# DaehwanKimLab/hisat2

Hardware: AMD Instinct MI355X
Metric: reads/sec, 101 bp PE, REDUCED-SIZE (256000000 bp, GRCh38 contig profile) linear index, --no-spliced-alignment: HI_Aligner::go per pair on the GPU (inputs and report events resident in HBM), SAM-identical to hisat2 (higher is better)
Workload: dtype u32

## Files before the change

### hisat2_amd/csrc/h2g_fast.h

```cpp
#pragma once
#include "h2g_align.h"
#ifndef FG_GRAPH
#define FG_GRAPH 0
#endif
#if FG_GRAPH
#include "h2g_graph.h"
#endif
#ifndef FG_SPLICED
#define FG_SPLICED 0
#endif
#if FG_SPLICED && (FG_GRAPH || FG_ALIGN_MATE)
#error "FG_SPLICED is built for linear indexes, without alignMate in the pass"
#endif

namespace h2g {

#define FG_FE     4
#define FG_HW     (6 + FG_FE / 2 + FG_GRAPH * FG_FE)
#define FG_LW     3
#define FG_NLONG  3
#define FG_NLONGC 3
#define FG_NLONGT (FG_NLONG + FG_NLONGC)
#define FG_NCO    5
#define FG_NRES   2
// ... 129 lines not shown
#define F_SMIN16 (-32768)
#define F_SMAX16 32767
H2G_HD uint32_t fs_rl(const FState& S, uint32_t m) { return m ? S.rl1 : S.rl0; }
H2G_HD uint32_t fs_ro(const FState& S, uint32_t m) { return m ? S.ro1 : S.ro0; }
H2G_HD uint32_t fs_nres(const FState& S, uint32_t m) { return m ? S.nres1 : S.nres0; }
H2G_HD uint32_t fs_nsearched(const FState& S, uint32_t m) { return m ? S.nsearched1 : S.nsearched0; }
H2G_HD int32_t fs_bestUnp(const FState& S, uint32_t m) { return m ? S.bestUnp1 : S.bestUnp0; }
H2G_HD int32_t fs_minsc(const FState& S, uint32_t m) { return m ? S.minsc1 : S.minsc0; }
H2G_HD uint32_t fs_b4(uint32_t w, uint32_t x) { return (w >> (8 * x)) & 0xffu; }
H2G_HD uint32_t fs_b4_set(uint32_t w, uint32_t x, uint32_t v) { return (w & ~(0xffu << (8 * x))) | ((v & 0xffu) << (8 * x)); }
H2G_HD uint32_t fs_sumsq(const FState& S, uint32_t x) { return x == 0 ? S.rb_sumsq0 : x == 1 ? S.rb_sumsq1 : x == 2 ? S.rb_sumsq2 : S.rb_sumsq3; }
H2G_HD void fs_sumsq_add(FState& S, uint32_t x, uint32_t v) { if(x == 0) S.rb_sumsq0 += v; else if(x == 1) S.rb_sumsq1 += v; else if(x == 2) S.rb_sumsq2 += v; else S.rb_sumsq3 += v; }
#define F_SMIN INT32_MIN

struct FCtx {
	const DGfm* g; const DRef* ref; const DLocalSet* ls; const AlnParams* P;
	DReads rd[2];
	const uint32_t* pk[2]; uint32_t pk_stride;
	const char* name[2]; uint32_t namelen[2];
	int64_t* sc; uint32_t sc_stride;
	FastOut O;
	uint32_t defer_slow = 0;
	uint32_t mate_handover = 0;
#if FG_GRAPH
	const DAlts* alts;
	GraphWS* gws;
#endif
#if FG_SPLICED
	const DSpliceDB* ssdb = nullptr;
	uint32_t rdid_base = 0;
#endif
};
#if FG_GRAPH
#define FG_IE_NOFIT 0xffffffffu
H2G_HD uint32_t fg_ie_pack(const IEdges& ie) {
	if(ie.n > 2) return FG_IE_NOFIT;
	uint32_t w = ie.n;
	if(ie.n > 0) { if(ie.e[0][0] > 127 || ie.e[0][1] > 127) return FG_IE_NOFIT; w |= (ie.e[0][0] << 2) | (ie.e[0][1] << 9); }
	if(ie.n > 1) { if(ie.e[1][0] > 127 || ie.e[1][1] > 127) return FG_IE_NOFIT; w |= (ie.e[1][0] << 16) | (ie.e[1][1] << 23); }
	return w;
}
H2G_HD void fg_ie_unpack(uint32_t w, IEdges* ie) {
	ie->n = w & 3u;
	ie->e[0][0] = (w >> 2) & 127u; ie->e[0][1] = (w >> 9) & 127u;
	ie->e[1][0] = (w >> 16) & 127u; ie->e[1][1] = (w >> 23) & 127u;
}
// ... 512 lines not shown
	const uint32_t ro = rd.offs[i], rl = rd.offs[i + 1] - ro;
	if(rl > H2G_PK_MAXLEN) return false;
	const uint8_t* src = rd.codes + ro;
	uint32_t anyn = 0;
	for(uint32_t w = 0; w < H2G_PK_WORDS; w++) {
		uint32_t bits = 0;
		if(w * 16 < rl) {
			for(uint32_t q = 0; q < 4; q++) {
				const uint32_t at = w * 16 + q * 4;
				if(at >= rl) break;
				uint32_t four;
				memcpy(&four, src + at, 4);
				const uint32_t left = rl - at;
				if(left < 4) four &= (1u << (8 * left)) - 1u;
				anyn |= four & 0x04040404u;
				const uint32_t lo = four & 0x03030303u;
				bits |= ((lo | (lo >> 6) | (lo >> 12) | (lo >> 18)) & 0xffu) << (8 * q);
			}
		}
		pk[w * stride] = bits;
	}
	return anyn == 0;
}
H2G_HD uint32_t fg_res_base(uint32_t m, uint32_t k) { return FW_RES + (m * FG_NRES + k) * 3; }
H2G_HD uint32_t fg_res_hit(uint32_t m, uint32_t k) { return FW_RH + (m * FG_NRES + k) * FG_HW; }

H2G_HD uint32_t fg_rand_seed(const FCtx& C, const FState& S, uint32_t set) {
	uint32_t rseed = C.P->seed0;
	const uint32_t len = fs_rl(S, set);
	const uint32_t* pk = set ? C.pk[1] : C.pk[0];
	for(uint32_t w = 0; w < H2G_PK_WORDS; w++) rseed ^= pk[w * C.pk_stride];
	const char* quals = set ? C.rd[1].quals : C.rd[0].quals;
	if(quals) {
		const char* q = quals + fs_ro(S, set);
		for(uint32_t i = 0; i < len; i++) rseed ^= ((uint32_t)q[i] << ((i & 3) << 3));
	} else {
		for(uint32_t b = 0; b < 4; b++) if(((len + 3 - b) >> 2) & 1u) rseed ^= (uint32_t)'I' << (b << 3);
	}
	const char* name = set ? C.name[1] : C.name[0];
	const uint32_t namelen = set ? C.namelen[1] : C.namelen[0];
	for(uint32_t i = 0; i < namelen; i++) {
		const int p = name[i];
		if(p == '/') break;
		rseed ^= ((uint32_t)p << ((i & 3) << 3));
	}
	return rseed;
// ... 155 lines not shown
		if(rdi < 0) F_GOTO(FPC_AFTER_LOOP);
		const uint32_t x = (uint32_t)rdi * 2 + (uint32_t)fwi, xr = (uint32_t)rdi * 2 + (uint32_t)(1 - fwi);
		{
			const uint32_t numSearched = fs_b4(S.rb_nps, x) - fs_b4(S.rb_nus, x);
			const int32_t bestScore = fs_bestUnp(S, rdi), msc = fs_minsc(S, rdi);
			if(bestScore >= msc) {
				const uint32_t maxmm = (uint32_t)((-(int64_t)bestScore + sc.mmpMax - 1) / sc.mmpMax);
				if(numSearched > maxmm + 1) {
					S.rb_done |= 1u << x; fg_pool_free(W, S, x);
					if(S.paired) {
						const int32_t ob = fs_bestUnp(S, 1 - rdi), om = fs_minsc(S, 1 - rdi);
						if(ob >= om && S.npairs > 0) F_GOTO(FPC_AFTER_LOOP); else F_GOTO(FPC_NB_PICK);
					} else F_GOTO(FPC_AFTER_LOOP);
				}
			}
			if(((S.rb_done >> xr) & 1u) && bestScore < msc) {
				const uint32_t rcs = fs_b4(S.rb_nps, xr) - fs_b4(S.rb_nus, xr);
				if(numSearched > rcs + (P.anchorStop ? 1u : 0u)) { S.rb_done |= 1u << x; fg_pool_free(W, S, x); F_GOTO(FPC_AFTER_LOOP); }
			}
		}
		S.nb_rdi = rdi; S.nb_fwi = fwi;
		S.sv_rdi = (uint32_t)rdi; S.sv_fw = fwi == 0;
		S.a0 = fs_b4(S.rb_cur, x);
		F_OP(FOP_PSEARCH, FPC_NB_AFTER_PS);
	}
	case FPC_NB_AFTER_PS: {
		const int rdi = S.nb_rdi, fwi = S.nb_fwi;
		const uint32_t x = (uint32_t)rdi * 2 + (uint32_t)fwi;
		const uint32_t top = S.a0, bot = S.a1, len = S.a2 & 0xffu, type = (S.a2 >> 8) & 0xffu, done = (S.a2 >> 16) & 1u, anchor = (S.a2 >> 17) & 1u, nus = S.a2 >> 18;
		{ const uint32_t nr_ = S.nrank + (S.a4 & 0xffffu), ns_ = S.nside + (S.a4 >> 16); if(nr_ > 0xffffu || ns_ > 0xffffu) F_BAIL(FB_OTHER); S.nrank = nr_; S.nside = ns_; }
		S.rb_nps = fs_b4_set(S.rb_nps, x, fs_b4(S.rb_nps, x) + 1); S.rb_nus = fs_b4_set(S.rb_nus, x, fs_b4(S.rb_nus, x) + nus); S.rb_cur = fs_b4_set(S.rb_cur, x, S.a3);
		const uint32_t np = fs_b4(S.rb_np, x);
		if(np >= 16) F_BAIL(FB_PARTIAL);
		fs_sumsq_add(S, x, len * len);
		if(bot > top && bot != H2G_MAX) {
			S.rb_nonempty |= 1u << x;
			if(len > minK + 2) {
				uint32_t k = 0;
				for(; k < FG_NLONG; k++) if(W.ld(FW_LONG + FG_LW * k + 2) == 0) break;
				if(k >= FG_NLONG) {
					for(; k < FG_NLONGT; k++) if(!((S.pool_x >> (k - FG_NLONG)) & 1u)) break;
					if(k >= FG_NLONGT) F_BAIL(FB_LONGPOOL);
					S.pool_x = S.pool_x | (1u << (k - FG_NLONG));
				}
				W.st(fg_pool(k), top); W.st(fg_pool(k) + 1, bot);
#if FG_GRAPH
// ... 1031 lines not shown
	case FPC_DONE:
	case FPC_BAIL:
	default: return;
	}
}
#undef F_GOTO
#undef F_OP
#undef F_RC_RET
#undef F_RC_CALL
#undef F_MINSC_LIVE

H2G_HD void fast_op_psearch(const FCtx& C, FState& S) {
	const AlnParams& P = *C.P;
	h2g_fm_hit fh;
#if FG_GRAPH
	IEdges ie;
	partial_search_graph_item(*C.g, fg_sv(C, S), S.a0, P.pseudogeneStop != 0, P.anchorStop != 0, P.khits, P.kseeds, &fh, &ie);
	S.a6 = fh.node_top; S.a7 = fh.node_bot; S.a8 = fg_ie_pack(ie);
#else
	partial_search_item(*C.g, fg_sv(C, S), S.a0, P.pseudogeneStop != 0, P.anchorStop != 0, P.khits, &fh);
#endif
	S.a5 = S.a0;
	S.a0 = fh.top; S.a1 = fh.bot;
	S.a2 = (fh.len & 0xffu) | (fh.hit_type << 8) | ((fh.done ? 1u : 0u) << 16) | ((fh.anchorStop ? 1u : 0u) << 17) | (fh.numUniqueSearch << 18);
	S.a3 = fh.cur; S.a4 = (fh.nrank & 0xffffu) | (fh.nside << 16);
}
#ifndef FG_WALK_STEPS
#define FG_WALK_STEPS 20
#endif
#ifndef FG_LWALK_STEPS
#define FG_LWALK_STEPS 10
#endif
#if FG_GRAPH
H2G_HD bool fast_op_gcoords(const FCtx& C, FState& S, const FWords& W) {
	if(!(S.a4 & 2u)) {
		uint32_t nelt = S.a7 - S.a6;
		if(nelt > S.a2) nelt = S.a2;
		if(nelt == 1 && S.a1 - S.a0 == 1) { S.a4 |= 2u; S.a2 = 0; }
	}
	if(S.a4 & 2u) {
		uint32_t row = S.a0, node = S.a6, steps = S.a2, off = 0;
		const uint32_t before = steps;
		const bool found = gw_walk_single(*C.g, &row, &node, &steps, FG_WALK_STEPS, &off);
		S.nsteps += steps - before;
		if(!found) {
			if(steps > 60000u) { S.pc = FPC_BAIL; S.bail = FB_GWALK; return false; }
			S.a0 = row; S.a6 = node; S.a2 = steps;
// ... 501 lines not shown
```

### hisat2_amd/csrc/h2g_go_args.h

```cpp
#pragma once
#include <hip/hip_runtime.h>
#include <atomic>
#include "h2g_align.h"
#include "h2g_graph.h"
#include "h2g_fast.h"

enum : unsigned {
	H2G_CNT_RANK = 0, H2G_CNT_SIDE = 1, H2G_CNT_STEPS = 2, H2G_CNT_EXT = 3,
	H2G_CNT_ALIGNED = 4, H2G_CNT_OVERFLOW = 5,
	H2G_CNT_FAST_DONE = 6, H2G_CNT_FAST_BAILED = 7,
	H2G_CNT_BENCH_SUM = 6, H2G_CNT_BENCH_CHECKSUM = 7,
	H2G_CNT_WORK_FAST = 12, H2G_CNT_WORK_DRAIN = 13, H2G_CNT_WORK_MAIN = 14, H2G_CNT_WORK_SECOND = 15,
	H2G_CNT_PROF_GO = 16, H2G_CNT_PROF_GO_CTL = 80,
	H2G_CNT_NO_SECOND = 64,
	H2G_CNT_FAST_BAIL_WHY = 96,
	H2G_CNT_FAST_RANK = 120, H2G_CNT_FAST_SIDE = 121, H2G_CNT_FAST_STEPS = 122, H2G_CNT_FAST_ALIGNED = 123,
	H2G_CNT_DRAIN_OFF = 120,
	H2G_CNT_OVF_CURSOR = 124, H2G_CNT_LEDITS_CURSOR = 126,
	H2G_CNT_PROF_FAST = 128, H2G_CNT_PROF_FAST_SITE = 176, H2G_CNT_PROF_FAST_TRIPS = 208,
	H2G_CNT_SECOND = 256,
	H2G_CNT_PROF_FAST_BINS = 512,
#ifdef H2G_GO_PROF
	H2G_CNT_BLOCK = 1024
#else
// ... 128 lines not shown
	h2g::DGfm g; h2g::DRef ref; h2g::DLocalSet ls;
	h2g::DReads rd1, rd2;
	h2g::AlnParams P;
	const char* names1; const uint32_t* noffs1;
	const char* names2; const uint32_t* noffs2;
	uint32_t* slots;
	h2g::FastOut O;
	unsigned long long* counters;
	uint32_t* work;
	uint32_t* bail_list; uint32_t* bail_count;
	uint32_t total, paired;
	h2g::DAlts alts;
	uint8_t* gws_base; size_t gws_stride;
	uint8_t* sc_base;
	uint32_t tail;
	uint32_t dbg_read; uint32_t* dbg_buf;
	uint32_t orphan_T; uint32_t* orphan_list; uint32_t* orphan_count;
	const uint32_t* adopt_list; const uint32_t* adopt_count; const uint32_t* adopt_slots;
	uint32_t cnt_off;
	uint32_t adopt_slot_words;
	uint32_t mate_handover;
	h2g::DSpliceDB ssdb;
	uint32_t rdid_base;
};
struct FastUnitDesc {
	int (*launch)(const FastArgs* a, unsigned grid, hipStream_t);
	int (*launch_drain)(const FastArgs* a, unsigned grid, hipStream_t);
	uint32_t threads, lds_bytes;
	uint32_t slots, slot_bytes;
	uint32_t gws_bytes;
};
extern "C" const FastUnitDesc* h2g_go_fast_unit();
extern "C" const FastUnitDesc* h2g_go_fast_am_unit();
extern "C" const FastUnitDesc* h2g_go_fast_graph_unit();
extern "C" const FastUnitDesc* h2g_go_fast_spl_unit();
```

### hisat2_amd/csrc/h2g_k_go_fast.hip

```cpp
#include "h2g_go_args.h"
#include "h2g_fast_prof.h"

using namespace h2g;

#ifndef FG_KERNEL
#define FG_KERNEL   k_go_fast
#define FG_UNIT     h2g_go_fast_unit
#endif
#define FG_CAT_(a, b) a##b
#define FG_CAT(a, b) FG_CAT_(a, b)
#define FG_KERNEL_DRAIN FG_CAT(FG_KERNEL, _drain)

#ifndef H2G_FAST_THREADS
#define H2G_FAST_THREADS 512
#endif
#ifndef H2G_FAST_SLOTS
#define H2G_FAST_SLOTS 1024
#endif
#ifndef FG_GWS_PRIVATE
#define FG_GWS_PRIVATE FG_GRAPH
#endif
#define FG_STAGE_WORDS (FW_HOT + 2 * H2G_PK_WORDS)
#define FG_SLOT_WORDS  (((FS_WORDS + FW_HOT + 2 * H2G_PK_WORDS + FW_COLD) + 3) & ~3)
#define FG_NQ ((int)FQ_COUNT)
// ... 7 lines not shown
__device__ __forceinline__ void fk_ctx(const FastArgs* A, uint32_t* stage, uint32_t* sm, FCtx& C, FWords& W) {
	const bool paired = A->paired != 0;
	W.hot = (FG_LDS uint32_t*)stage; W.hot_stride = H2G_FAST_THREADS; W.cold = sm + FS_WORDS + FG_STAGE_WORDS;
	uint32_t* const pk0 = stage + FW_HOT * H2G_FAST_THREADS;
	C.g = &A->g; C.ref = &A->ref; C.ls = &A->ls; C.P = &A->P;
	C.rd[0] = A->rd1; C.rd[1] = paired ? A->rd2 : A->rd1;
	C.pk[0] = pk0; C.pk[1] = paired ? pk0 + H2G_PK_WORDS * H2G_FAST_THREADS : pk0; C.pk_stride = H2G_FAST_THREADS;
	C.sc = nullptr; C.sc_stride = 0;
#if FG_GRAPH
	{
		const size_t tid = (size_t)blockIdx.x * H2G_FAST_THREADS + threadIdx.x;
		C.alts = &A->alts;
#if !FG_GWS_PRIVATE
		C.gws = reinterpret_cast<GraphWS*>(A->gws_base + tid * A->gws_stride);
#endif
		C.sc = reinterpret_cast<int64_t*>(A->sc_base + (tid >> 6) * (size_t)(64 * 2 * H2G_COMBINE_MAXLEN * sizeof(int64_t))) + (threadIdx.x & 63); C.sc_stride = 64;
	}
#endif
#if FG_SPLICED
	C.ssdb = &A->ssdb; C.rdid_base = A->rdid_base;
#endif
	C.O = A->O;
	C.mate_handover = FG_ALIGN_MATE ? 0u : A->mate_handover;
	C.defer_slow = FG_GRAPH ? 1u : 0u;
	C.name[0] = C.name[1] = nullptr; C.namelen[0] = C.namelen[1] = 0;
}
__device__ __forceinline__ void fk_load_state(FState& S, const uint32_t* sm) {
	uint32_t w[FS_WORDS];
	const uint4* src = reinterpret_cast<const uint4*>(sm);
#pragma unroll
	for(uint32_t k = 0; k < FS_WORDS / 4; k++) { const uint4 v = src[k]; w[4 * k] = v.x; w[4 * k + 1] = v.y; w[4 * k + 2] = v.z; w[4 * k + 3] = v.w; }
	__builtin_memcpy(&S, w, sizeof S);
}
__device__ __forceinline__ void fk_store_state(const FState& S, uint32_t* sm) {
	uint32_t w[FS_WORDS];
	__builtin_memcpy(w, &S, sizeof S);
	uint4* dst = reinterpret_cast<uint4*>(sm);
#pragma unroll
	for(uint32_t k = 0; k < FS_WORDS / 4; k++) dst[k] = make_uint4(w[4 * k], w[4 * k + 1], w[4 * k + 2], w[4 * k + 3]);
}
__device__ __forceinline__ void fk_trip(const FastArgs* A, uint32_t* stage, uint32_t* sm, FState& S, uint32_t op, uint32_t begin, uint32_t packed_ok) {
	FCtx C; FWords W;
	fk_ctx(A, stage, sm, C, W);
#if FG_GRAPH && FG_GWS_PRIVATE
	GraphWS gws_private;
	C.gws = &gws_private;
// ... 261 lines not shown
```

### hisat2_amd/csrc/h2g_kernels.hip

```cpp
#include <hip/hip_runtime.h>
#include <stdio.h>
#include <stdlib.h>
#include <string>
#include <vector>
#include <thread>
#include <atomic>
#include <memory>
#include <chrono>
#include <algorithm>
#define H2G_EXT_OPTS 0
#define H2G_HAPLOTYPE 0
#include "h2g_core.h"
#include "h2g_dev.h"
#include "h2g_host_index.h"
#include "h2g_align.h"
#include "h2g_graph.h"
#include "h2g_sw.h"
#include "h2g_graph_staged.h"
#include "h2g_local_pack.h"
#include "h2g_splice_host.h"
#include "h2g_splice_db_host.h"
#include "h2g_windows.h"
#include "h2g_fastq.h"
#include "h2g_sam_line.h"
// ... 58 lines not shown
	return g;
}

static DLocalSet dls_now(h2g_index* ix) {
	DLocalSet l = ix->dls;
	if(!ix->d_lsa) return l;
	if(!ix->lsa_ready.load(std::memory_order_acquire)) {
		if(hipEventQuery(ix->lsa_ev) != hipSuccess) { (void)hipGetLastError(); return l; }
		ix->lsa_ready.store(true, std::memory_order_release);
	}
	l.lsa = ix->d_lsa; l.lsa_base = ix->d_lsa_base;
	return l;
}

#define H2G_MSTREAMS_MAX 8
#define H2G_MSTREAMS_LIGHT_DEFAULT 2
#define H2G_NBUF (H2G_MSTREAMS_MAX + 1)
#define H2G_FAST_RESERVE_DEFAULT 0
#define H2G_DEFAULT_TAIL 16
#define H2G_ORPHAN_T 512
#define H2G_ORPHAN_MIN_UNITS 200000
#define H2G_DRAIN_GRID 64
#define H2G_FAST_POOLS 3
#define H2G_DEFAULT_ALIGN_MATE 0
#define H2G_DEFAULT_FAST_SPLICED 0
#define H2G_MACH_MAXGRID 48u
#define H2G_MACH_TOTAL 128u
#define H2G_MAX_BATCHES 16
struct BatchCtx {
	size_t n_reads = 0; uint32_t max_read_len = 0;
	DevBuf<uint8_t> d_codes; DevBuf<uint32_t> d_offs; DevBuf<char> d_quals; bool has_quals = false;
	DevBuf<char> d_names; DevBuf<uint32_t> d_name_offs; bool has_names = false;
	DevBuf<uint8_t> d_codes2; DevBuf<uint32_t> d_offs2; DevBuf<char> d_quals2, d_names2; DevBuf<uint32_t> d_name_offs2; bool has_mates = false, has_quals2 = false;
	DevBuf<ReadOut> d_rout; DevBuf<h2g_alnres> d_aln; uint32_t aln_slots = 0;
	DevBuf<PairOut> d_pout; DevBuf<h2g_alnres> d_paln[2]; uint32_t pair_slots = 0;
	DevBuf<uint32_t> d_seeds; bool has_seeds = false, has_seeds2 = false;
	DevBuf<uint8_t> d_qc; bool has_qc = false;
	DevBuf<uint32_t> d_ids; bool has_ids = false;
	hipError_t ensure_reads(size_t max_reads, size_t max_bases) {
		hipError_t e = d_codes.ensure(max_bases + 64);
		if(e == hipSuccess) e = d_quals.ensure(max_bases + 64);
		return e != hipSuccess ? e : d_offs.ensure(max_reads + 1);
	}
	hipError_t reserve_names(size_t nb, size_t max_reads) {
		if(d_names.size() >= nb + 64 && d_name_offs) return hipSuccess;
		const hipError_t e = d_names.reset(nb + 64);
// ... 24 lines not shown
	unsigned long long* cnt_cur = nullptr;
	uint32_t last_bails = 0;
	PinnedBuf<uint32_t> h_bails;
	size_t max_reads = 0, max_bases = 0;
	BatchCtx batch[H2G_MAX_BATCHES];
	unsigned cur_batch = 0;
	BatchCtx& cur() { return batch[cur_batch]; }
	const BatchCtx& cur() const { return batch[cur_batch]; }
	DevBuf<h2g_seed_result> d_seed;
	struct GoPool {
		DevBuf<uint8_t> ws;
		DevBuf<uint8_t> gws;
		DevBuf<uint8_t> sw; size_t sw_stride = 0, sw_lanes = 0;
		DevBuf<uint8_t> sc;
	} pool[2 * H2G_MSTREAMS_MAX];
	DevBuf<uint32_t> dbg_buf;
	DevBuf<uint32_t> d_ovf_list[H2G_MSTREAMS_MAX];
	unsigned ovf_cur = 0;
	DevBuf<uint32_t> d_bail_list[H2G_NBUF];
	DevBuf<FastArgs> d_fast_args[2 * H2G_NBUF];
	PinnedBuf<FastArgs> h_fast_args;
	DevBuf<uint8_t> d_fast_slots[H2G_FAST_POOLS];
	DevEvent ev_pool[H2G_FAST_POOLS];
	DevBuf<uint32_t> d_orphans[H2G_NBUF];
	size_t orphan_cap = 0;
	DevBuf<uint8_t> d_drain_slots;
	DevBuf<uint8_t> d_drain_sc;
	DevEvent ev_drain[H2G_NBUF];
	bool dst_busy = false;
	DevEvent ev_bails[H2G_NBUF];
	DevEvent ev_dr[2];
	bool ran_drain = false;
	const uint32_t* orph_cur = nullptr;
	DevBuf<uint8_t> d_fast_gws;
	DevBuf<uint8_t> d_fast_sc;
	bool ran_fast = false;
	struct Tune { int fast = 1, blocks_per_cu = 0, pair_slots = 0, no_second_pass = 0; unsigned mach_div = 0 , mach_min = 4, mach_total = H2G_MACH_TOTAL; int mach_total_auto = 1; int fast_reserve = H2G_FAST_RESERVE_DEFAULT; long dbg_read = -1;
	              int tail = H2G_DEFAULT_TAIL, tail_auto = 1, align_mate = H2G_DEFAULT_ALIGN_MATE; int orphan = -1 , drain_grid = H2G_DRAIN_GRID, mate_handover = -1 ;
	              int fast_spliced = H2G_DEFAULT_FAST_SPLICED;  } tune;
	h2g_align_params last_p; int last_paired = -1;
	DevBuf<uint8_t> d_sw_ws;
	DevBuf<SwLaneState> d_sw_states;
	DevBuf<h2g_edit> d_ledits; DevBuf<uint32_t> d_ledits_cur; size_t ledits_cap = 0; unsigned ledits_parts = 0;
	unsigned ledits_touched = 0;
	DevBuf<h2g_alnres> d_paln_ovf; size_t paln_ovf_cap = 0; unsigned paln_ovf_parts = 0;
	DevBuf<uint32_t> d_xlp_at, d_xlp; size_t xlp_cap = 0; unsigned xlp_parts = 0; DevBuf<uint32_t> d_xlp_cur;
	const PairOut* xlp_pout = nullptr;
	DevBuf<unsigned long long> d_counters;
	DevBuf<uint8_t> d_tmp[4];
	uint64_t tmp_gen = 0;
	struct CompactFetch { bool valid = false, paired = false; uint64_t gen = 0; unsigned batch = 0; size_t first = 0, n = 0; const uint8_t* d_rec[2] = {nullptr, nullptr}; uint64_t bytes[2] = {0, 0};
	                      const uint64_t* d_boffs[2] = {nullptr, nullptr};  } cfetch;
	DevBuf<uint8_t> d_sam[5];
	uint64_t samtab_uid = 0, samtab_gen = 0; uint32_t samtab_nrefs = 0, samtab_names = 0, samtab_rg = 0, samtab_nalts = 0; int32_t samtab_strand = 0;
	DevEvent ev_sam[4];
	h2g_sam_text_stats sam_stats = {};
	DevBuf<uint8_t> d_plan[5];
	DevEvent ev_plan[4];
	h2g_sam_plan_stats plan_stats = {};
	std::vector<uint8_t> plan_classes;
	DevEvent ev[14];
// ... 574 lines not shown
	for(int k = 0; k < H2G_MSTREAMS_MAX; k++) { HIPCHK(s->mst[k].create(hipStreamNonBlocking)); HIPCHK(s->ev_rot[k].create(hipEventDisableTiming)); }
	HIPCHK(s->dst.create(hipStreamNonBlocking));
	HIPCHK(s->h_fast_args.ensure(2 * H2G_NBUF));
	HIPCHK(s->h_bails.ensure(H2G_NBUF)); for(int k = 0; k < H2G_NBUF; k++) s->h_bails[k] = 0;
	for(int k = 0; k < H2G_NBUF; k++) { HIPCHK(s->ev_fast[k].create(hipEventDisableTiming)); HIPCHK(s->ev_mach[k].create(hipEventDisableTiming)); HIPCHK(s->ev_bails[k].create(hipEventDisableTiming)); HIPCHK(s->ev_drain[k].create(hipEventDisableTiming)); }
	for(int k = 0; k < H2G_FAST_POOLS; k++) HIPCHK(s->ev_pool[k].create(hipEventDisableTiming));
	for(int k = 0; k < 2; k++) HIPCHK(s->ev_dr[k].create());
	for(int i = 0; i < 14; i++) HIPCHK(s->ev[i].create());
	HIPCHK(s->d_counters.ensure(H2G_NBUF * H2G_CNT_BLOCK));
	HIPCHK(hipMemset(s->d_counters, 0, s->d_counters.bytes()));
	s->cnt_cur = s->d_counters;
	if(max_reads) {
		HIPCHK(s->batch[0].ensure_reads(max_reads, max_bases));
		HIPCHK(s->d_seed.ensure(max_reads * 2));
		HIPCHK(hipMemset(s->d_seed, 0, s->d_seed.bytes()));
	}
	memset(&s->last, 0, sizeof s->last);
	{
		auto env = [](const char* k, long d) { const char* e = getenv(k); return e ? atol(e) : d; };
		s->tune.fast = (int)env("H2G_GO_FAST", 1); s->tune.blocks_per_cu = (int)env("H2G_GO_BLOCKS_PER_CU", 0); s->tune.pair_slots = (int)env("H2G_PAIR_SLOTS", 0);
		s->tune.no_second_pass = (int)env("H2G_GO_NO_SECOND_PASS", 0); s->tune.mach_div = (unsigned)env("H2G_MACH_DIV", 0); s->tune.mach_min = (unsigned)env("H2G_MACH_MIN", 4);
		s->tune.dbg_read = env("H2G_GO_DBG_READ", -1);
		s->tune.tail = (int)env("H2G_FAST_TAIL", H2G_DEFAULT_TAIL); s->tune.tail_auto = getenv("H2G_FAST_TAIL") ? 0 : 1; s->tune.align_mate = (int)env("H2G_FAST_AM", H2G_DEFAULT_ALIGN_MATE);
		s->tune.orphan = (int)env("H2G_FAST_ORPHAN", -1); s->tune.drain_grid = (int)env("H2G_DRAIN_GRID", H2G_DRAIN_GRID); s->tune.mate_handover = (int)env("H2G_FAST_MATE_HANDOVER", -1);
		s->tune.fast_spliced = (int)env("H2G_FAST_SPLICED", H2G_DEFAULT_FAST_SPLICED);
		s->tune.mach_total = (unsigned)env("H2G_MACH_TOTAL", H2G_MACH_TOTAL); s->tune.mach_total_auto = getenv("H2G_MACH_TOTAL") ? 0 : 1; s->tune.fast_reserve = (int)env("H2G_FAST_RESERVE", H2G_FAST_RESERVE_DEFAULT);
		auto clampm = [](long m) { return (unsigned)(m < 1 ? 1 : m > H2G_MSTREAMS_MAX ? H2G_MSTREAMS_MAX : m); };
		if(getenv("H2G_MSTREAMS")) s->mstreams = clampm(env("H2G_MSTREAMS", 0));
		s->mstreams_light = clampm(env("H2G_MSTREAMS_LIGHT", H2G_MSTREAMS_LIGHT_DEFAULT));
	}
	*out = sp.release();
	return H2G_OK;
}

extern "C" void h2g_stream_free(h2g_stream* s) { delete s; }

static hipError_t sync_mach(h2g_stream* s) {
	if(!s->st2_busy) return hipSuccess;
	for(unsigned k = 0; k < s->n_mst; k++) { const hipError_t e = hipStreamSynchronize(s->mst[k]); if(e != hipSuccess) return e; }
	s->st2_busy = false;
	return hipSuccess;
}
static hipError_t sync_all(h2g_stream* s) {
	hipError_t e = hipStreamSynchronize(s->st);
	if(e == hipSuccess && s->dst_busy) { e = hipStreamSynchronize(s->dst); s->dst_busy = false; }
	if(e == hipSuccess && s->st2_busy) { e = sync_mach(s); s->st2_busy = false; }
	return e;
// ... 1498 lines not shown
	if(s->tune.blocks_per_cu > 0) per_cu = (size_t)s->tune.blocks_per_cu;
	const size_t want = (n_reads + g->U->slots - 1) / g->U->slots;
	size_t maxblocks = 256 * per_cu;
	if(g->big_main && maxblocks > 32) maxblocks = 32;
	if(g->xl && maxblocks > 12) maxblocks = 12;
	g->grid = (unsigned)(want < 1 ? 1 : (want > maxblocks ? maxblocks : want));
	g->M = s->mstreams ? s->mstreams : H2G_MSTREAMS_MAX;
	const bool mt_auto = s->tune.mach_total_auto != 0 && g->linear;
	g->units = paired ? n_reads : (n_reads + 1) / 2;
	const unsigned mach_total_now = mt_auto && (size_t)s->last_bails * 1000 > g->units * 15 ? 192u : s->tune.mach_total;
	g->S = mstreams_policy(g->units, s->last_bails, g->linear, s->mstreams, s->mstreams_light);
	g->mach_cap = mach_total_now / g->M;
	if(g->mach_cap > H2G_MACH_MAXGRID) g->mach_cap = H2G_MACH_MAXGRID;
	if(g->mach_cap < 1) g->mach_cap = 1;
	g->pool_cap = (mt_auto ? 192u : s->tune.mach_total) / g->M;
	if(g->pool_cap > H2G_MACH_MAXGRID) g->pool_cap = H2G_MACH_MAXGRID;
	if(g->pool_cap < g->mach_cap) g->pool_cap = g->mach_cap;
	g->bgrid = g->fast ? 2u : 4u;
	return plan;
}

struct FastPlan {
	bool use_am, mate_ho;
	const FastUnitDesc *FU, *DU;
	unsigned fgrid, mgrid, dgrid;
	uint32_t orphan_T, psel;
	size_t slot_bytes;
};
struct GoRun {
	GoArgs A; DExonTbl X; XlPairs XP;
	unsigned gsel, msel, ssel;
	unsigned long long* cblk;
	FastPlan f;
	hipStream_t ms;
	unsigned mach_grid, psel, qsel;
	uint32_t* ovl;
};

static void go_args(const h2g_stream* s, const h2g_align_params* p, bool paired, const GoPlan& g, GoRun* r) {
	const BatchCtx& b = s->cur();
	GoArgs& A = r->A;
	memset(&A, 0, sizeof A);
	A.g = dg_now(s->ix); A.ref = s->ix->dr; A.ls = dls_now(s->ix); A.alts = s->ix->dalts;
	if(p->max_alts_tried) A.alts.maxAltsTried = p->max_alts_tried;
	if(p->use_haplotype && !g.linear && A.alts.n) A.alts.has_splice |= 2u;
	A.rd1 = dreads(s); A.rd2 = A.rd1;
// ... 127 lines not shown
		mach_div = 400;
		if(!linear) {
			const size_t units = paired ? n_reads : n_reads / 2;
			if(units >= 1000000) mach_div = 1600;
			else if(units > 500000) mach_div = 400 + (unsigned)((units - 500000) * 1200 / 500000);
		}
	}
	f->mgrid = (unsigned)((s->last_bails + mach_div - 1) / (mach_div ? mach_div : 1u));
	if(f->mgrid < s->tune.mach_min) f->mgrid = s->tune.mach_min;
	if(f->mgrid > g.mach_cap) f->mgrid = g.mach_cap;
	const size_t fwant = (n_reads + 127) / 128;
	unsigned reserve = s->tune.fast_reserve >= 0 ? (unsigned)s->tune.fast_reserve : g.S * f->mgrid;
	if(reserve > 192) reserve = 192;
	const unsigned fmax = 256 - reserve;
	f->fgrid = (unsigned)(fwant < 1 ? 1 : (fwant > fmax ? fmax : fwant));
	f->slot_bytes = (size_t)256 * f->FU->slots * f->FU->slot_bytes;
	f->orphan_T = s->tune.orphan >= 0 ? (uint32_t)s->tune.orphan : (g.units >= H2G_ORPHAN_MIN_UNITS ? (uint32_t)H2G_ORPHAN_T : 0u);
	if(f->orphan_T > f->FU->slots) f->orphan_T = f->FU->slots;
	if(f->FU->gws_bytes != 0) f->orphan_T = 0;
	f->dgrid = (unsigned)(s->tune.drain_grid < 1 ? 1 : s->tune.drain_grid);
	f->mate_ho = f->orphan_T != 0 && linear && paired && !f->use_am && !g.fast_spl && s->tune.mate_handover != 0;
	f->DU = &fast_unit(linear, g.fast_spl, f->use_am || f->mate_ho);
	f->psel = f->orphan_T ? s->gen % H2G_FAST_POOLS : 0u;
}

static int fast_buffers(h2g_stream* s, const GoPlan& g, const FastPlan& f) {
	const size_t ocap = (size_t)256 * f.FU->slots, dbytes = (size_t)f.dgrid * f.DU->slots * f.DU->slot_bytes;
	const size_t dsc = g.linear ? 0 : (size_t)f.dgrid * f.FU->threads * (size_t)(2 * H2G_COMBINE_MAXLEN * sizeof(int64_t));
	bool need = s->d_fast_slots[f.psel].size() < f.slot_bytes;
	if(f.orphan_T) {
		for(unsigned q = 0; q < H2G_FAST_POOLS; q++) need = need || s->d_fast_slots[q].size() < f.slot_bytes;
		need = need || s->d_drain_slots.size() < dbytes || s->d_drain_sc.size() < dsc;
		for(unsigned b = 0; b < g.M + 1; b++) need = need || !s->d_orphans[b] || !s->d_fast_args[H2G_NBUF + b];
		need = need || s->orphan_cap < ocap;
	}
	if(!need) return H2G_OK;
	HIPCHK(hipStreamSynchronize(s->st)); HIPCHK(hipStreamSynchronize(s->dst)); for(unsigned k = 0; k < s->n_mst; k++) HIPCHK(hipStreamSynchronize(s->mst[k]));
	for(unsigned q = 0; q < (f.orphan_T ? (unsigned)H2G_FAST_POOLS : 1u); q++) {
		DevBuf<uint8_t>& fs = s->d_fast_slots[f.orphan_T ? q : f.psel];
		if(fs.size() < f.slot_bytes) { HIPCHK(fs.reserve(f.slot_bytes)); HIPCHK(hipMemsetAsync(fs, 0, f.slot_bytes, s->st)); }
	}
	if(f.orphan_T) {
		if(s->orphan_cap < ocap) { for(int b = 0; b < H2G_NBUF; b++) s->d_orphans[b] = DevBuf<uint32_t>(); s->orphan_cap = ocap; }
		for(unsigned b = 0; b < g.M + 1; b++) {
			if(!s->d_orphans[b]) { HIPCHK(s->d_orphans[b].ensure(s->orphan_cap + 4)); HIPCHK(hipMemsetAsync(s->d_orphans[b], 0, (s->orphan_cap + 4) * 4, s->st)); }
			HIPCHK(s->d_fast_args[H2G_NBUF + b].ensure(1));
		}
		if(s->d_drain_slots.size() < dbytes) { HIPCHK(s->d_drain_slots.reserve(dbytes)); HIPCHK(hipMemsetAsync(s->d_drain_slots, 0, dbytes, s->st)); }
		if(s->d_drain_sc.size() < dsc) { HIPCHK(s->d_drain_sc.reserve(dsc)); HIPCHK(hipMemsetAsync(s->d_drain_sc, 0, dsc, s->st)); }
	}
	HIPCHK(hipStreamSynchronize(s->st));
	return H2G_OK;
}

static int fast_launch(h2g_stream* s, bool paired, const GoPlan& g, GoRun* r) {
	const FastPlan& f = r->f;
	const GoArgs& A = r->A;
	const unsigned gsel = r->gsel;
	HIPCHK(hipStreamWaitEvent(s->st, s->ev_pool[f.psel], 0));
	HIPCHK(s->d_bail_list[gsel].ensure(s->max_reads + 4));
	uint32_t* const bl = s->d_bail_list[gsel];
	HIPCHK(hipMemsetAsync(bl + s->max_reads, 0, 16, s->st));
	FastArgs F;
	memset(&F, 0, sizeof F);
	F.g = A.g; F.ref = A.ref; F.ls = A.ls; F.rd1 = A.rd1; F.rd2 = A.rd2; F.P = A.P;
	F.names1 = A.names1; F.noffs1 = A.noffs1; F.names2 = A.names2; F.noffs2 = A.noffs2;
	F.slots = (uint32_t*)s->d_fast_slots[f.psel].get();
	F.O.rout = A.O.rout; F.O.aln = A.O.aln; F.O.aln_slots = A.O.aln_slots; F.O.pout = A.O.pout; F.O.paln[0] = A.O.paln[0]; F.O.paln[1] = A.O.paln[1]; F.O.pair_slots = A.O.pair_slots;
	F.counters = r->cblk; F.work = reinterpret_cast<uint32_t*>(r->cblk + H2G_CNT_WORK_FAST);
	F.bail_list = bl; F.bail_count = bl + s->max_reads;
	F.total = (uint32_t)s->cur().n_reads; F.paired = paired ? 1u : 0u;
	F.alts = A.alts; F.gws_base = nullptr; F.gws_stride = 0; F.sc_base = nullptr;
	F.dbg_read = A.dbg_read; F.dbg_buf = A.dbg_buf;
	F.ssdb = A.ssdb; F.rdid_base = A.rdid_base;
	F.tail = g.linear && paired && s->tune.tail > 0 ? (uint32_t)s->tune.tail : 0u;
	if(!g.linear) {
		const size_t lanes = (size_t)256 * f.FU->threads;
		HIPCHK(s->d_fast_gws.reserve(lanes * f.FU->gws_bytes));
		HIPCHK(s->d_fast_sc.reserve(lanes * (size_t)(2 * H2G_COMBINE_MAXLEN * sizeof(int64_t))));
		F.gws_base = s->d_fast_gws; F.gws_stride = f.FU->gws_bytes; F.sc_base = s->d_fast_sc;
	}
	HIPCHK(s->d_fast_args[gsel].ensure(1));
	FastArgs D = F;
	if(f.orphan_T) {
		uint32_t* const ol = s->d_orphans[gsel];
		HIPCHK(hipMemsetAsync(ol + s->orphan_cap, 0, 16, s->st));
		F.orphan_T = f.orphan_T; F.orphan_list = ol; F.orphan_count = ol + s->orphan_cap; F.mate_handover = f.mate_ho ? 1u : 0u;
		D.adopt_slot_words = f.FU->slot_bytes / 4;
		if(s->tune.tail_auto) D.tail = g.linear && paired && (size_t)s->last_bails * 1000 > g.units * 15 ? (uint32_t)H2G_DEFAULT_TAIL : 0u;
		D.slots = (uint32_t*)s->d_drain_slots.get();
		D.adopt_list = ol; D.adopt_count = ol + s->orphan_cap; D.adopt_slots = F.slots;
		D.work = reinterpret_cast<uint32_t*>(r->cblk + H2G_CNT_WORK_DRAIN);
		D.cnt_off = H2G_CNT_DRAIN_OFF;
		D.total = 0;
		if(!g.linear) D.sc_base = s->d_drain_sc;
		s->orph_cur = ol + s->orphan_cap;
	}
	if(s->gen >= g.M + 1 && hipEventQuery(s->ev_fast[gsel]) != hipSuccess) { (void)hipGetLastError(); HIPCHK(hipEventSynchronize(s->ev_fast[gsel])); }
	FastArgs* const hF = s->h_fast_args + gsel;
	*hF = F;
	HIPCHK(hipMemcpyAsync(s->d_fast_args[gsel], hF, sizeof F, hipMemcpyHostToDevice, s->st));
	if(f.orphan_T) {
		FastArgs* const hD = s->h_fast_args + H2G_NBUF + gsel;
		*hD = D;
		HIPCHK(hipMemcpyAsync(s->d_fast_args[H2G_NBUF + gsel], hD, sizeof D, hipMemcpyHostToDevice, s->st));
	}
	if(f.FU->launch(s->d_fast_args[gsel], f.fgrid, s->st) != 0) return set_err("go() fast pass launch", hipGetLastError());
	r->A.list = bl; r->A.nlist = bl + s->max_reads;
	return H2G_OK;
}

static int fast_handoff(h2g_stream* s, bool paired, const GoPlan& g, GoRun* r) {
	const FastPlan& f = r->f;
	const unsigned gsel = r->gsel;
	HIPCHK(hipEventRecord(s->ev_fast[gsel], s->st));
	r->ms = s->mst[r->ssel]; s->st2_busy = true;
	if(f.mgrid < r->mach_grid) r->mach_grid = f.mgrid;
	if(f.orphan_T) {
		HIPCHK(hipStreamWaitEvent(s->dst, s->ev_fast[gsel], 0));
		HIPCHK(hipEventRecord(s->ev_dr[0], s->dst));
		if(f.DU->launch_drain(s->d_fast_args[H2G_NBUF + gsel], f.dgrid, s->dst) != 0) return set_err("go() drain launch", hipGetLastError());
		HIPCHK(hipEventRecord(s->ev_dr[1], s->dst));
		HIPCHK(hipEventRecord(s->ev_pool[f.psel], s->dst));
		HIPCHK(hipMemcpyAsync(&s->h_bails[gsel], s->d_bail_list[gsel] + s->max_reads, 4, hipMemcpyDeviceToHost, s->dst));
		HIPCHK(hipEventRecord(s->ev_drain[gsel], s->dst));
		HIPCHK(hipEventRecord(s->ev_bails[gsel], s->dst));
		HIPCHK(hipStreamWaitEvent(r->ms, s->ev_drain[gsel], 0));
		s->ran_drain = true; s->dst_busy = true;
	} else {
// ... 1025 lines not shown
	}
	*n = hi;
	if(hi == 0) return H2G_OK;
	if(!out || cap < hi) return H2G_ERR_ARG;
	for(unsigned m = 0; m < s->ledits_parts; m++) {
		size_t end = cur[m]; const size_t lo = m * s->ledits_cap, top = (m + 1) * s->ledits_cap;
		if(end > top) end = top;
		if(end > lo) HIPCHK(hipMemcpy(out + lo, s->d_ledits + lo, (end - lo) * sizeof(h2g_edit), hipMemcpyDeviceToHost));
	}
	return H2G_OK;
}

extern "C" __attribute__((visibility("default"))) int h2g_stream_tune(h2g_stream* s, const char* key, long v) {
	if(!s || !key) return H2G_ERR_ARG;
	HIPCHK(sync_all(s));
	for(unsigned k_ = 0; k_ < s->n_mst; k_++) HIPCHK(hipStreamSynchronize(s->mst[k_]));
	const std::string k(key);
	if(k == "fast") s->tune.fast = (int)v; else if(k == "blocks_per_cu") s->tune.blocks_per_cu = (int)v; else if(k == "pair_slots") s->tune.pair_slots = (int)v;
	else if(k == "no_second_pass") s->tune.no_second_pass = (int)v; else if(k == "mach_div") s->tune.mach_div = (unsigned)v; else if(k == "mach_min") s->tune.mach_min = (unsigned)v;
	else if(k == "dbg_read") s->tune.dbg_read = v; else if(k == "tail") { s->tune.tail = (int)v; s->tune.tail_auto = 0; } else if(k == "align_mate") s->tune.align_mate = (int)v;
	else if(k == "mach_total") { s->tune.mach_total_auto = v <= 0; s->tune.mach_total = v <= 0 ? H2G_MACH_TOTAL : (unsigned)v; }
	else if(k == "fast_reserve") s->tune.fast_reserve = (int)v;
	else if(k == "mate_handover") s->tune.mate_handover = (int)v;
	else if(k == "fast_spliced") s->tune.fast_spliced = (int)v;
	else if(k == "orphan") s->tune.orphan = (int)v; else if(k == "drain_grid") s->tune.drain_grid = (int)(v < 1 ? 1 : v > 128 ? 128 : v);
	else if(k == "mstreams") { s->mstreams = (unsigned)(v < 1 ? 1 : v > H2G_MSTREAMS_MAX ? H2G_MSTREAMS_MAX : v); s->gen = 0; }
	else if(k == "mstreams_light") s->mstreams_light = (unsigned)(v < 1 ? 1 : v > H2G_MSTREAMS_MAX ? H2G_MSTREAMS_MAX : v);
	else return H2G_ERR_ARG;
	return H2G_OK;
}

extern "C" __attribute__((visibility("default"))) long h2g_stream_probe(const h2g_stream* s, const char* key) {
	if(!s || !key) return -1;
	const std::string k(key);
	if(k == "mstreams_rotation") return (long)s->rot;
	if(k == "mstreams_used") return (long)s->n_mst;
	if(k == "mstreams_created") { long n = 0; for(hipStream_t m : s->mst) n += m != nullptr; return n; }
	if(k == "lanes") return (long)(s->mstreams ? s->mstreams : H2G_MSTREAMS_MAX);
	if(k == "pools") { long n = 0; for(const h2g_stream::GoPool& pl : s->pool) n += bool(pl.ws); return n; }
	return -1;
}

extern "C" __attribute__((visibility("default"))) int h2g_go_debug_trace(h2g_stream* s, uint32_t* out, uint32_t cap_words) {
	if(s) HIPCHK(sync_mach(s));
	if(!s || !out || !s->dbg_buf) return H2G_ERR_ARG;
	HIPCHK(sync_all(s));
// ... 74 lines not shown
```

Before: 212.4 million.

## Precompute first partial search per read/strand in a dense pre-pass kernel

Adds a separate kernel that, before the fast pass, runs the first partial FM-index search (offset 0) for every read, mate and strand, one lane per search, and stores a compact 4-word record. The fast-pass state machine then loads this record instead of running the search when the cursor is zero, skipping divergent per-thread FM walks inside the large, register-heavy state-machine kernel. This costs an extra launch, a buffer of max_reads*16 words per pool, and duplicate read packing, and nrank/nside are truncated to 12 bits in the packed record. It is enabled by default for linear, non-spliced indexes.

```diff
diff --git a/hisat2_amd/csrc/h2g_fast.h b/hisat2_amd/csrc/h2g_fast.h
--- a/hisat2_amd/csrc/h2g_fast.h
+++ b/hisat2_amd/csrc/h2g_fast.h
@@ -175,6 +175,7 @@
 	FastOut O;
 	uint32_t defer_slow = 0;
 	uint32_t mate_handover = 0;
+	const uint32_t* ps0 = nullptr;
 #if FG_GRAPH
 	const DAlts* alts;
 	GraphWS* gws;
@@ -733,6 +734,26 @@
 	}
 	return anyn == 0;
 }
+#define FG_PS0_WORDS 4
+#define FG_PS0_ABSENT 0xffffffffu
+H2G_HD uint32_t fg_ps_a2(const h2g_fm_hit& fh) {
+	return (fh.len & 0xffu) | (fh.hit_type << 8) | ((fh.done ? 1u : 0u) << 16) | ((fh.anchorStop ? 1u : 0u) << 17) | (fh.numUniqueSearch << 18);
+}
+H2G_HD void fg_ps0_pack(const h2g_fm_hit& fh, uint32_t rec[FG_PS0_WORDS]) {
+	rec[0] = fh.top; rec[1] = fh.bot; rec[2] = fg_ps_a2(fh); rec[3] = (fh.cur & 0xffu) | ((fh.nrank & 0xfffu) << 8) | ((fh.nside & 0xfffu) << 20);
+}
+H2G_HD bool fg_ps0_load(const uint32_t* tbl, uint32_t read, uint32_t x, FState& S) {
+	const uint32_t* p = tbl + ((size_t)read * 4 + x) * FG_PS0_WORDS;
+	uint32_t r0, r1, r2, r3;
+#if defined(__HIP_DEVICE_COMPILE__)
+	{ const uint4 v = *reinterpret_cast<const uint4*>(p); r0 = v.x; r1 = v.y; r2 = v.z; r3 = v.w; }
+#else
+	r0 = p[0]; r1 = p[1]; r2 = p[2]; r3 = p[3];
+#endif
+	if(r3 == FG_PS0_ABSENT) return false;
+	S.a0 = r0; S.a1 = r1; S.a2 = r2; S.a3 = r3 & 0xffu; S.a4 = ((r3 >> 8) & 0xfffu) | ((r3 >> 20) << 16); S.a5 = 0;
+	return true;
+}
 H2G_HD uint32_t fg_res_base(uint32_t m, uint32_t k) { return FW_RES + (m * FG_NRES + k) * 3; }
 H2G_HD uint32_t fg_res_hit(uint32_t m, uint32_t k) { return FW_RH + (m * FG_NRES + k) * FG_HW; }
 
@@ -934,6 +955,9 @@
 		S.nb_rdi = rdi; S.nb_fwi = fwi;
 		S.sv_rdi = (uint32_t)rdi; S.sv_fw = fwi == 0;
 		S.a0 = fs_b4(S.rb_cur, x);
+#if !FG_GRAPH && !FG_SPLICED
+		if(C.ps0 && S.a0 == 0 && fg_ps0_load(C.ps0, S.read, x, S)) F_GOTO(FPC_NB_AFTER_PS);
+#endif
 		F_OP(FOP_PSEARCH, FPC_NB_AFTER_PS);
 	}
 	case FPC_NB_AFTER_PS: {
@@ -2011,7 +2035,7 @@
 #endif
 	S.a5 = S.a0;
 	S.a0 = fh.top; S.a1 = fh.bot;
-	S.a2 = (fh.len & 0xffu) | (fh.hit_type << 8) | ((fh.done ? 1u : 0u) << 16) | ((fh.anchorStop ? 1u : 0u) << 17) | (fh.numUniqueSearch << 18);
+	S.a2 = fg_ps_a2(fh);
 	S.a3 = fh.cur; S.a4 = (fh.nrank & 0xffffu) | (fh.nside << 16);
 }
 #ifndef FG_WALK_STEPS
diff --git a/hisat2_amd/csrc/h2g_go_args.h b/hisat2_amd/csrc/h2g_go_args.h
--- a/hisat2_amd/csrc/h2g_go_args.h
+++ b/hisat2_amd/csrc/h2g_go_args.h
@@ -174,7 +174,9 @@
 	uint32_t mate_handover;
 	h2g::DSpliceDB ssdb;
 	uint32_t rdid_base;
+	uint32_t* ps0;
 };
+extern "C" int h2g_ps0_launch(const FastArgs* a, uint32_t units, bool paired, hipStream_t st);
 struct FastUnitDesc {
 	int (*launch)(const FastArgs* a, unsigned grid, hipStream_t);
 	int (*launch_drain)(const FastArgs* a, unsigned grid, hipStream_t);
diff --git a/hisat2_amd/csrc/h2g_k_go_fast.hip b/hisat2_amd/csrc/h2g_k_go_fast.hip
--- a/hisat2_amd/csrc/h2g_k_go_fast.hip
+++ b/hisat2_amd/csrc/h2g_k_go_fast.hip
@@ -53,6 +53,7 @@
 #endif
 	C.O = A->O;
 	C.mate_handover = FG_ALIGN_MATE ? 0u : A->mate_handover;
+	C.ps0 = A->ps0;
 	C.defer_slow = FG_GRAPH ? 1u : 0u;
 	C.name[0] = C.name[1] = nullptr; C.namelen[0] = C.namelen[1] = 0;
 }
diff --git a/hisat2_amd/csrc/h2g_k_ps0.hip b/hisat2_amd/csrc/h2g_k_ps0.hip
--- /dev/null
+++ b/hisat2_amd/csrc/h2g_k_ps0.hip
@@ -0,0 +1,48 @@
+#include "h2g_go_args.h"
+
+using namespace h2g;
+
+#define PS0_THREADS 256
+
+__global__ __launch_bounds__(PS0_THREADS, 6) void k_ps0(const FastArgs* __restrict__ A, uint32_t units)
+{
+	__shared__ uint32_t s_pk[H2G_PK_WORDS * PS0_THREADS];
+	const bool paired = A->paired != 0;
+	const uint32_t sh = paired ? 2u : 1u;
+	const uint32_t t = blockIdx.x * PS0_THREADS + threadIdx.x;
+	const uint32_t unit = t >> sh, x = t & ((1u << sh) - 1u), mate = x >> 1;
+	const uint32_t lane = threadIdx.x & 63u;
+	const bool live = unit < units;
+	const DReads& rd = mate ? A->rd2 : A->rd1;
+	uint32_t* const pk = s_pk + (threadIdx.x & ~1u);
+	bool ok = true;
+	uint32_t rl = 0;
+	if(live) {
+		rl = rd.offs[unit + 1] - rd.offs[unit];
+		if((x & 1u) == 0) {
+			ok = fg_pack_read(rd, unit, pk, PS0_THREADS);
+			if(rd.qc && !rd.qc[unit]) ok = false;
+		}
+	}
+	__syncthreads();
+	const unsigned long long bad = __ballot(!ok);
+	const bool absent = ((bad >> (lane & ~((1u << sh) - 1u))) & ((1ull << (1u << sh)) - 1ull)) != 0;
+	if(!live) return;
+	uint32_t rec[FG_PS0_WORDS] = {FG_PS0_ABSENT, FG_PS0_ABSENT, FG_PS0_ABSENT, FG_PS0_ABSENT};
+	if(!absent) {
+		SeqView sv;
+		sv.fwc = nullptr; sv.q = nullptr; sv.len = rl; sv.fw = (x & 1u) == 0;
+		sv.pk = pk; sv.pk_stride = PS0_THREADS; sv.pk_nomask = true;
+		h2g_fm_hit fh;
+		partial_search_item(A->g, sv, 0, A->P.pseudogeneStop != 0, A->P.anchorStop != 0, A->P.khits, &fh);
+		fg_ps0_pack(fh, rec);
+	}
+	*reinterpret_cast<uint4*>(A->ps0 + ((size_t)unit * 4 + x) * FG_PS0_WORDS) = make_uint4(rec[0], rec[1], rec[2], rec[3]);
+}
+
+extern "C" int h2g_ps0_launch(const FastArgs* a, uint32_t units, bool paired, hipStream_t st) {
+	if(units == 0) return 0;
+	const unsigned long long lanes = (unsigned long long)units * (paired ? 4u : 2u);
+	hipLaunchKernelGGL(k_ps0, dim3((unsigned)((lanes + PS0_THREADS - 1) / PS0_THREADS)), dim3(PS0_THREADS), 0, st, a, units);
+	return (int)hipGetLastError();
+}
diff --git a/hisat2_amd/csrc/h2g_kernels.hip b/hisat2_amd/csrc/h2g_kernels.hip
--- a/hisat2_amd/csrc/h2g_kernels.hip
+++ b/hisat2_amd/csrc/h2g_kernels.hip
@@ -104,6 +104,9 @@
 #define H2G_ORPHAN_MIN_UNITS 200000
 #define H2G_DRAIN_GRID 64
 #define H2G_FAST_POOLS 3
+#ifndef H2G_DEFAULT_PS0
+#define H2G_DEFAULT_PS0 1
+#endif
 #define H2G_DEFAULT_ALIGN_MATE 0
 #define H2G_DEFAULT_FAST_SPLICED 0
 #define H2G_MACH_MAXGRID 48u
@@ -174,6 +177,7 @@
 	PinnedBuf<FastArgs> h_fast_args;
 	DevBuf<uint8_t> d_fast_slots[H2G_FAST_POOLS];
 	DevEvent ev_pool[H2G_FAST_POOLS];
+	DevBuf<uint32_t> d_ps0[H2G_FAST_POOLS];
 	DevBuf<uint32_t> d_orphans[H2G_NBUF];
 	size_t orphan_cap = 0;
 	DevBuf<uint8_t> d_drain_slots;
@@ -189,6 +193,7 @@
 	bool ran_fast = false;
 	struct Tune { int fast = 1, blocks_per_cu = 0, pair_slots = 0, no_second_pass = 0; unsigned mach_div = 0 , mach_min = 4, mach_total = H2G_MACH_TOTAL; int mach_total_auto = 1; int fast_reserve = H2G_FAST_RESERVE_DEFAULT; long dbg_read = -1;
 	              int tail = H2G_DEFAULT_TAIL, tail_auto = 1, align_mate = H2G_DEFAULT_ALIGN_MATE; int orphan = -1 , drain_grid = H2G_DRAIN_GRID, mate_handover = -1 ;
+	              int ps0 = -1;
 	              int fast_spliced = H2G_DEFAULT_FAST_SPLICED;  } tune;
 	h2g_align_params last_p; int last_paired = -1;
 	DevBuf<uint8_t> d_sw_ws;
@@ -809,7 +814,7 @@
 		s->tune.no_second_pass = (int)env("H2G_GO_NO_SECOND_PASS", 0); s->tune.mach_div = (unsigned)env("H2G_MACH_DIV", 0); s->tune.mach_min = (unsigned)env("H2G_MACH_MIN", 4);
 		s->tune.dbg_read = env("H2G_GO_DBG_READ", -1);
 		s->tune.tail = (int)env("H2G_FAST_TAIL", H2G_DEFAULT_TAIL); s->tune.tail_auto = getenv("H2G_FAST_TAIL") ? 0 : 1; s->tune.align_mate = (int)env("H2G_FAST_AM", H2G_DEFAULT_ALIGN_MATE);
-		s->tune.orphan = (int)env("H2G_FAST_ORPHAN", -1); s->tune.drain_grid = (int)env("H2G_DRAIN_GRID", H2G_DRAIN_GRID); s->tune.mate_handover = (int)env("H2G_FAST_MATE_HANDOVER", -1);
+		s->tune.orphan = (int)env("H2G_FAST_ORPHAN", -1); s->tune.drain_grid = (int)env("H2G_DRAIN_GRID", H2G_DRAIN_GRID); s->tune.mate_handover = (int)env("H2G_FAST_MATE_HANDOVER", -1); s->tune.ps0 = (int)env("H2G_FAST_PS0", -1);
 		s->tune.fast_spliced = (int)env("H2G_FAST_SPLICED", H2G_DEFAULT_FAST_SPLICED);
 		s->tune.mach_total = (unsigned)env("H2G_MACH_TOTAL", H2G_MACH_TOTAL); s->tune.mach_total_auto = getenv("H2G_MACH_TOTAL") ? 0 : 1; s->tune.fast_reserve = (int)env("H2G_FAST_RESERVE", H2G_FAST_RESERVE_DEFAULT);
 		auto clampm = [](long m) { return (unsigned)(m < 1 ? 1 : m > H2G_MSTREAMS_MAX ? H2G_MSTREAMS_MAX : m); };
@@ -2354,6 +2359,7 @@
 
 struct FastPlan {
 	bool use_am, mate_ho;
+	bool ps0;
 	const FastUnitDesc *FU, *DU;
 	unsigned fgrid, mgrid, dgrid;
 	uint32_t orphan_T, psel;
@@ -2527,6 +2533,7 @@
 	f->mate_ho = f->orphan_T != 0 && linear && paired && !f->use_am && !g.fast_spl && s->tune.mate_handover != 0;
 	f->DU = &fast_unit(linear, g.fast_spl, f->use_am || f->mate_ho);
 	f->psel = f->orphan_T ? s->gen % H2G_FAST_POOLS : 0u;
+	f->ps0 = linear && !g.fast_spl && (s->tune.ps0 < 0 ? H2G_DEFAULT_PS0 != 0 : s->tune.ps0 != 0);
 }
 
 static int fast_buffers(h2g_stream* s, const GoPlan& g, const FastPlan& f) {
@@ -2539,11 +2546,15 @@
 		for(unsigned b = 0; b < g.M + 1; b++) need = need || !s->d_orphans[b] || !s->d_fast_args[H2G_NBUF + b];
 		need = need || s->orphan_cap < ocap;
 	}
+	const size_t pswords = (size_t)s->max_reads * 4 * FG_PS0_WORDS;
+	if(f.ps0) for(unsigned q = 0; q < (f.orphan_T ? (unsigned)H2G_FAST_POOLS : 1u); q++) need = need || s->d_ps0[f.orphan_T ? q : f.psel].size() < pswords;
 	if(!need) return H2G_OK;
 	HIPCHK(hipStreamSynchronize(s->st)); HIPCHK(hipStreamSynchronize(s->dst)); for(unsigned k = 0; k < s->n_mst; k++) HIPCHK(hipStreamSynchronize(s->mst[k]));
 	for(unsigned q = 0; q < (f.orphan_T ? (unsigned)H2G_FAST_POOLS : 1u); q++) {
 		DevBuf<uint8_t>& fs = s->d_fast_slots[f.orphan_T ? q : f.psel];
 		if(fs.size() < f.slot_bytes) { HIPCHK(fs.reserve(f.slot_bytes)); HIPCHK(hipMemsetAsync(fs, 0, f.slot_bytes, s->st)); }
+		DevBuf<uint32_t>& ps = s->d_ps0[f.orphan_T ? q : f.psel];
+		if(f.ps0 && ps.size() < pswords) { HIPCHK(ps.reserve(pswords)); HIPCHK(hipMemsetAsync(ps, 0xff, pswords * 4, s->st)); }
 	}
 	if(f.orphan_T) {
 		if(s->orphan_cap < ocap) { for(int b = 0; b < H2G_NBUF; b++) s->d_orphans[b] = DevBuf<uint32_t>(); s->orphan_cap = ocap; }
@@ -2577,6 +2588,7 @@
 	F.total = (uint32_t)s->cur().n_reads; F.paired = paired ? 1u : 0u;
 	F.alts = A.alts; F.gws_base = nullptr; F.gws_stride = 0; F.sc_base = nullptr;
 	F.dbg_read = A.dbg_read; F.dbg_buf = A.dbg_buf;
+	F.ps0 = f.ps0 ? s->d_ps0[f.psel].get() : nullptr;
 	F.ssdb = A.ssdb; F.rdid_base = A.rdid_base;
 	F.tail = g.linear && paired && s->tune.tail > 0 ? (uint32_t)s->tune.tail : 0u;
 	if(!g.linear) {
@@ -2610,6 +2622,7 @@
 		*hD = D;
 		HIPCHK(hipMemcpyAsync(s->d_fast_args[H2G_NBUF + gsel], hD, sizeof D, hipMemcpyHostToDevice, s->st));
 	}
+	if(f.ps0 && h2g_ps0_launch(s->d_fast_args[gsel], F.total, paired, s->st) != 0) return set_err("go() first-search pre-pass launch", hipGetLastError());
 	if(f.FU->launch(s->d_fast_args[gsel], f.fgrid, s->st) != 0) return set_err("go() fast pass launch", hipGetLastError());
 	r->A.list = bl; r->A.nlist = bl + s->max_reads;
 	return H2G_OK;
@@ -3681,6 +3694,7 @@
 	else if(k == "mach_total") { s->tune.mach_total_auto = v <= 0; s->tune.mach_total = v <= 0 ? H2G_MACH_TOTAL : (unsigned)v; }
 	else if(k == "fast_reserve") s->tune.fast_reserve = (int)v;
 	else if(k == "mate_handover") s->tune.mate_handover = (int)v;
+	else if(k == "ps0") s->tune.ps0 = (int)v;
 	else if(k == "fast_spliced") s->tune.fast_spliced = (int)v;
 	else if(k == "orphan") s->tune.orphan = (int)v; else if(k == "drain_grid") s->tune.drain_grid = (int)(v < 1 ? 1 : v > 128 ? 128 : v);
 	else if(k == "mstreams") { s->mstreams = (unsigned)(v < 1 ? 1 : v > H2G_MSTREAMS_MAX ? H2G_MSTREAMS_MAX : v); s->gen = 0; }
```

New measurement: 221.5 million (median of 6 runs). +4.3%, better.
